# succinctlabs/sp1

Hardware: NVIDIA H100
Metric: riscv_cycles_proven_per_second_core (higher is better)
Workload: dtype u32 KoalaBear (Montgomery) / ext4

## Files before the change

sp1_b200/csrc/hostcheck.cu:

```cuda
#include "poseidon2.cuh"
#include "hostfield.hpp"
#include "zc_lower.hpp"
#include <cstring>
#include <type_traits>

extern "C" {
void sp1b200_hostcheck_permute(uint32_t* states, uint64_t n) {
    for (uint64_t i = 0; i < n; i++) {
        uint32_t s[16];
        for (int k = 0; k < 16; k++) s[k] = states[i * 16 + k];
        p2::permute(s);
        for (int k = 0; k < 16; k++) states[i * 16 + k] = s[k];
    }
}
int sp1b200_hostcheck_permute_mode(uint32_t* states, uint64_t n, int mode) {
    for (uint64_t i = 0; i < n; i++) {
        uint32_t s[16];
        for (int k = 0; k < 16; k++) s[k] = states[i * 16 + k];
        switch (mode) {
#define P2_CASE(M) case M: p2::permute_m<M>(s); break;
            P2_CASE(0) P2_CASE(1) P2_CASE(2) P2_CASE(3) P2_CASE(4) P2_CASE(5) P2_CASE(6) P2_CASE(7)
            P2_CASE(8) P2_CASE(9) P2_CASE(10) P2_CASE(11) P2_CASE(12) P2_CASE(13) P2_CASE(14) P2_CASE(15)
            P2_CASE(19) P2_CASE(21) P2_CASE(23)
#undef P2_CASE
            case -1: p2::permute_r1(s); break;
            default: return 0;
        }
        for (int k = 0; k < 16; k++) states[i * 16 + k] = s[k];
    }
    return 1;
}
void sp1b200_hostcheck_ext_mul(const uint32_t* a, const uint32_t* b, uint32_t* out, uint64_t n) {
    for (uint64_t i = 0; i < n; i++) {
        kb::Ext x{{a[4 * i], a[4 * i + 1], a[4 * i + 2], a[4 * i + 3]}}, y{{b[4 * i], b[4 * i + 1], b[4 * i + 2], b[4 * i + 3]}};
        kb::Ext r = kb::ext_mul(x, y);
        for (int k = 0; k < 4; k++) out[4 * i + k] = r.c[k];
    }
}
void sp1b200_hostcheck_ext_inv(const uint32_t* a, uint32_t* out, uint64_t n) {
    for (uint64_t i = 0; i < n; i++) {
        kb::Ext x{{a[4 * i], a[4 * i + 1], a[4 * i + 2], a[4 * i + 3]}};
        kb::Ext r = kb::ext_inv(x);
        for (int k = 0; k < 4; k++) out[4 * i + k] = r.c[k];
    }
}
void sp1b200_hostcheck_field(const uint32_t* a, const uint32_t* b, uint32_t* add, uint32_t* sub, uint32_t* mul, uint64_t n) {
    for (uint64_t i = 0; i < n; i++) { add[i] = kb::add(a[i], b[i]); sub[i] = kb::sub(a[i], b[i]); mul[i] = kb::mul(a[i], b[i]); }
}

int sp1b200_hostcheck_zc_lower(const uint32_t* chip, const uint32_t* main_row, const uint32_t* prep_row, const uint32_t* pv,
                               const uint32_t* alpha_pows, uint32_t window, uint32_t* out, uint32_t* n_lowered) {
    using hf::E4;
    const uint32_t* b = chip;
    HostProg hp;
    b += 3;
    const uint32_t n_regs = *b++;
    const uint32_t ni = *b++, nl = *b++, nc = *b++, np = *b++, na = *b++;
    hp.instrs.resize(ni); memcpy(hp.instrs.data(), b, ni * 8); b += 2 * ni;
    hp.leaves.resize(nl); memcpy(hp.leaves.data(), b, nl * 8); b += 2 * nl;
    hp.consts.assign(b, b + nc); b += nc;
    hp.publics.assign(b, b + np); b += np;
    hp.assert_regs.assign(b, b + na); b += na;
    hp.assert_alphas.assign(b, b + na); b += na;
    auto leaf = [&](const LeafRef& l) { return l.source == LEAF_MAIN ? main_row[l.col] : prep_row[l.col]; };
    {
        std::vector<uint32_t> regs(n_regs ? n_regs : 1, 0);
        for (const DagInstr& in : hp.instrs) {
            switch (in.opcode) {
                case BC_LOAD_LEAF: regs[in.out] = leaf(hp.leaves[in.a]); break;
                case BC_LOAD_CONST: regs[in.out] = hp.consts[in.a]; break;
                case BC_LOAD_PUBLIC: regs[in.out] = pv[hp.publics[in.a]]; break;
                case BC_ADD_F: regs[in.out] = hf::add(regs[in.a], regs[in.b]); break;
                case BC_SUB_F: regs[in.out] = hf::sub(regs[in.a], regs[in.b]); break;
                case BC_MUL_F: regs[in.out] = hf::mul(regs[in.a], regs[in.b]); break;
                case BC_NEG_F: regs[in.out] = hf::neg(regs[in.a]); break;
            }
        }
        E4 acc;
        for (size_t k = 0; k < hp.assert_regs.size(); k++) acc = acc + E4::load(alpha_pows + 4 * hp.assert_alphas[k]) * regs[hp.assert_regs[k]];
        acc.store(out);
    }
    auto run = [&](const ZcLowered& Lw) {
        std::vector<uint32_t> rf(Lw.n_regs, 0);
        E4 a;
        for (const ZcInstr& in : Lw.instrs) {
            switch (in.op) {
                case ZC_LOAD_MAIN: rf[in.out] = main_row[(uint32_t)in.a | ((uint32_t)in.b << 16)]; break;
                case ZC_LOAD_PREP: rf[in.out] = prep_row[(uint32_t)in.a | ((uint32_t)in.b << 16)]; break;
                case ZC_CONST: rf[in.out] = hp.consts[in.a]; break;
                case ZC_PUBLIC: rf[in.out] = pv[hp.publics[in.a]]; break;
                case ZC_ADD: { uint32_t x = rf[in.a], y = rf[in.b]; rf[in.out] = hf::add(x, y); break; }
                case ZC_SUB: { uint32_t x = rf[in.a], y = rf[in.b]; rf[in.out] = hf::sub(x, y); break; }
                case ZC_MUL: { uint32_t x = rf[in.a], y = rf[in.b]; rf[in.out] = hf::mul(x, y); break; }
                case ZC_NEG: rf[in.out] = hf::neg(rf[in.a]); break;
                case ZC_ASSERT: a = a + E4::load(alpha_pows + 4 * in.b) * rf[in.a]; break;
            }
        }
        return a;
    };
    ZcLowered L = zc_lower(hp, window);
    if (!L.error.empty()) return -1;
    if (n_lowered) *n_lowered = (uint32_t)L.instrs.size();
    E4 acc = run(L);
    {
        const size_t na = hp.assert_regs.size();
        const size_t np_ = std::max<size_t>(1, std::min<size_t>(16, na / 4));
        E4 sum;
        for (size_t q = 0; q < np_; q++) {
            ZcLowered P = zc_lower(hp, window, na * q / np_, na * (q + 1) / np_);
            if (!P.error.empty() || P.n_regs > L.n_regs + 8) return -1;
            sum = sum + run(P);
        }
        sum.store(out + 8);
    }
    acc.store(out + 4);
    return (int)L.n_regs;
}

void sp1b200_hostcheck_e4(const uint32_t* a, const uint32_t* b, uint32_t* mul_out, uint32_t* inv_out, uint64_t n) {
    using hf::E4;
    for (uint64_t i = 0; i < n; i++) {
        (E4::load(a + 4 * i) * E4::load(b + 4 * i)).store(mul_out + 4 * i);
        hf::inv(E4::load(a + 4 * i)).store(inv_out + 4 * i);
    }
}
int sp1b200_hostcheck_interpolate(const uint32_t* xs, const uint32_t* ys, uint32_t n, uint32_t* coeffs_out) {
    using hf::E4;
    auto go = [&](auto tag) {
        constexpr int N = decltype(tag)::value;
        E4 x[N], L[N][N], c[N];
        for (int i = 0; i < N; i++) x[i] = E4::load(xs + 4 * i);
        hf::lagrange_basis<N>(x, L);
        for (int k = 0; k < N; k++) for (int i = 0; i < N; i++) c[k] = c[k] + L[i][k] * E4::load(ys + 4 * i);
        for (int k = 0; k < N; k++) c[k].store(coeffs_out + 4 * k);
    };
    if (n == 3) go(std::integral_constant<int, 3>{});
    else if (n == 4) go(std::integral_constant<int, 4>{});
    else if (n == 5) go(std::integral_constant<int, 5>{});
    else return -1;
    return 0;
}
}
```

sp1_b200/csrc/zc_lower.hpp:

```cpp
#pragma once
#include "machine.cuh"
#include <cstdint>
#include <functional>
#include <queue>
#include <string>
#include <vector>

enum : uint8_t { ZC_LOAD_MAIN = 0, ZC_LOAD_PREP = 1, ZC_CONST = 2, ZC_PUBLIC = 3, ZC_ADD = 4, ZC_SUB = 5, ZC_MUL = 6, ZC_NEG = 7, ZC_ASSERT = 8 };
struct ZcInstr { uint8_t op, pad; uint16_t out, a, b; };
static_assert(sizeof(ZcInstr) == 8, "ZcInstr is one 8-byte word");

struct ZcLowered { std::vector<ZcInstr> instrs; uint32_t n_regs = 0; std::string error; };

inline ZcLowered zc_lower(const HostProg& p, uint32_t window = 24, size_t assert_begin = 0, size_t assert_end = (size_t)-1) {
    ZcLowered L;
    const size_t n = p.instrs.size();
    const int32_t NONE = -1;
    std::vector<int32_t> cur(65536, NONE);
    std::vector<int32_t> va(n, NONE), vb(n, NONE);
    std::vector<uint8_t> is_op(n, 0), needed(n, 0);
    for (size_t i = 0; i < n; i++) {
        const DagInstr& in = p.instrs[i];
        switch (in.opcode) {
            case BC_LOAD_LEAF: case BC_LOAD_CONST: case BC_LOAD_PUBLIC: break;
            case BC_ADD_F: case BC_SUB_F: case BC_MUL_F:
                va[i] = cur[in.a]; vb[i] = cur[in.b]; is_op[i] = 1;
                if (va[i] == NONE || vb[i] == NONE) { L.error = "instruction reads an undefined register"; return L; }
                break;
            case BC_NEG_F:
                va[i] = cur[in.a]; is_op[i] = 1;
                if (va[i] == NONE) { L.error = "instruction reads an undefined register"; return L; }
                break;
            default: L.error = "unknown opcode"; return L;
        }
        cur[in.out] = (int32_t)i;
    }
    std::vector<std::vector<uint32_t>> asserts_of(n);
    if (assert_end > p.assert_regs.size()) assert_end = p.assert_regs.size();
    for (size_t k = assert_begin; k < assert_end; k++) {
        const int32_t v = cur[p.assert_regs[k] & 0xffff];
        if (v == NONE) { L.error = "assert on an undefined register"; return L; }
        if (p.assert_alphas[k] > 0xffff) { L.error = "more than 65536 constraints in one chip"; return L; }
        asserts_of[v].push_back(p.assert_alphas[k]);
        needed[v] = 1;
    }
    for (size_t i = n; i-- > 0;) {
        if (!needed[i]) continue;
        if (va[i] != NONE) needed[va[i]] = 1;
        if (vb[i] != NONE) needed[vb[i]] = 1;
    }
    std::vector<uint32_t> seq;
    for (size_t i = 0; i < n; i++) if (needed[i] && is_op[i]) seq.push_back((uint32_t)i);
    std::vector<std::vector<uint32_t>> uses(n);
    for (uint32_t pos = 0; pos < seq.size(); pos++) {
        const uint32_t i = seq[pos];
        if (va[i] != NONE) uses[va[i]].push_back(pos);
        if (vb[i] != NONE && vb[i] != va[i]) uses[vb[i]].push_back(pos);
    }
    std::vector<uint32_t> use_ptr(n, 0);
    std::vector<int32_t> reg_of(n, NONE);
    std::priority_queue<uint32_t, std::vector<uint32_t>, std::greater<uint32_t>> free_regs;
    uint32_t next_reg = 0;
    auto alloc = [&]() -> uint32_t {
        if (!free_regs.empty()) { uint32_t r = free_regs.top(); free_regs.pop(); return r; }
        return next_reg++;
    };
    auto emit_load = [&](uint32_t v, uint32_t r) {
        const DagInstr& in = p.instrs[v];
        ZcInstr z{};
        z.out = (uint16_t)r;
        if (in.opcode == BC_LOAD_LEAF) {
            const LeafRef& l = p.leaves[in.a];
            z.op = l.source == LEAF_MAIN ? ZC_LOAD_MAIN : ZC_LOAD_PREP;
            z.a = (uint16_t)(l.col & 0xffff); z.b = (uint16_t)(l.col >> 16);
        } else {
            z.op = in.opcode == BC_LOAD_CONST ? ZC_CONST : ZC_PUBLIC;
            z.a = in.a;
        }
        L.instrs.push_back(z);
    };
    auto operand = [&](int32_t v) -> uint32_t {
        if (reg_of[v] == NONE) {
            reg_of[v] = (int32_t)alloc();
            emit_load((uint32_t)v, (uint32_t)reg_of[v]);
        }
        return (uint32_t)reg_of[v];
    };
    auto release_after_use = [&](int32_t v, uint32_t pos) {
        std::vector<uint32_t>& u = uses[v];
        uint32_t& q = use_ptr[v];
        while (q < u.size() && u[q] <= pos) q++;
        const bool more = q < u.size();
        const bool keep = more && (is_op[v] || u[q] - pos <= window);
        if (!keep && reg_of[v] != NONE) { free_regs.push((uint32_t)reg_of[v]); reg_of[v] = NONE; }
    };
    for (uint32_t pos = 0; pos < seq.size(); pos++) {
        const uint32_t i = seq[pos];
        const DagInstr& in = p.instrs[i];
        const uint32_t ra = operand(va[i]);
        const uint32_t rb = vb[i] != NONE ? operand(vb[i]) : 0;
        release_after_use(va[i], pos);
        if (vb[i] != NONE && vb[i] != va[i]) release_after_use(vb[i], pos);
        const uint32_t ro = alloc();
        reg_of[i] = (int32_t)ro;
        ZcInstr z{};
        z.op = in.opcode == BC_ADD_F ? ZC_ADD : in.opcode == BC_SUB_F ? ZC_SUB : in.opcode == BC_MUL_F ? ZC_MUL : ZC_NEG;
        z.out = (uint16_t)ro; z.a = (uint16_t)ra; z.b = (uint16_t)rb;
        L.instrs.push_back(z);
        for (uint32_t alpha : asserts_of[i]) L.instrs.push_back(ZcInstr{ZC_ASSERT, 0, 0, (uint16_t)ro, (uint16_t)alpha});
        if (uses[i].empty()) { free_regs.push(ro); reg_of[i] = NONE; }
    }
    for (size_t v = 0; v < n; v++) {
        if (is_op[v] || asserts_of[v].empty()) continue;
        const uint32_t r = operand((int32_t)v);
        for (uint32_t alpha : asserts_of[v]) L.instrs.push_back(ZcInstr{ZC_ASSERT, 0, 0, (uint16_t)r, (uint16_t)alpha});
        free_regs.push(r); reg_of[v] = NONE;
    }
    if (next_reg > 0xffff) { L.error = "register pressure exceeds 65535"; return L; }
    L.n_regs = next_reg ? next_reg : 1;
    return L;
}
```

sp1_b200/csrc/zerocheck.cu:

```cuda
#include "ctx.cuh"
#include "challenger.cuh"
#include "hostfield.hpp"
#include "kb31.cuh"
#include <algorithm>
#include <memory>
#include <vector>

#include "machine.cuh"
#include "zc_lower.hpp"
#include "sumcheck.cuh"

namespace {

using kb::Ext;
using hf::E4;

constexpr int ZC_BLOCK = 128;
constexpr int ZC_LOCAL_REGS = 128;
constexpr int ZC_GLOBAL_REGS = 1024;
constexpr unsigned ZC_GLOBAL_MAXB = 132 * 2;
constexpr size_t ZC_MAX_PIECES = 16;

template <class K> struct Ops;
template <> struct Ops<uint32_t> {
    static __device__ __forceinline__ uint32_t zero() { return 0; }
    static __device__ __forceinline__ uint32_t from_base(uint32_t x) { return x; }
    static __device__ __forceinline__ uint32_t add(uint32_t a, uint32_t b) { return kb::add(a, b); }
    static __device__ __forceinline__ uint32_t sub(uint32_t a, uint32_t b) { return kb::sub(a, b); }
    static __device__ __forceinline__ uint32_t mul(uint32_t a, uint32_t b) { return kb::mul(a, b); }
    static __device__ __forceinline__ uint32_t load(const uint32_t* p, uint64_t i) { return __ldg(p + i); }
    static __device__ __forceinline__ Ext scale(const Ext& e, uint32_t k) { return kb::ext_mul_base(e, k); }
};
template <> struct Ops<Ext> {
    static __device__ __forceinline__ Ext zero() { return kb::ext_zero(); }
    static __device__ __forceinline__ Ext from_base(uint32_t x) { return kb::ext_from_base(x); }
    static __device__ __forceinline__ Ext add(const Ext& a, const Ext& b) { return kb::ext_add(a, b); }
    static __device__ __forceinline__ Ext sub(const Ext& a, const Ext& b) { return kb::ext_sub(a, b); }
    static __device__ __forceinline__ Ext mul(const Ext& a, const Ext& b) { return kb::ext_mul(a, b); }
    static __device__ __forceinline__ Ext load(const Ext* p, uint64_t i) { return kb::ext_load(reinterpret_cast<const uint32_t*>(p + i)); }
    static __device__ __forceinline__ Ext scale(const Ext& e, const Ext& k) { return kb::ext_mul(e, k); }
};

struct ZcJob {
    const void* main; const void* prep; const uint32_t* alpha_pows; uint64_t h;
    uint32_t blk_start, nblk, chip, columns;
    uint32_t zc_begin, zc_end;
    const void* batch;
};
static_assert(sizeof(ZcJob) == 64, "ZcJob layout");
struct ZcFixJob {
    const void* main; const void* prep; uint32_t* out; uint64_t h;
    uint32_t main_w, prep_w, blk_start, pad;
};

template <class J>
__device__ __forceinline__ int find_job(const J* __restrict__ jobs, int n, uint32_t blk) {
    int lo = 0, hi = n - 1;
    while (lo < hi) {
        int mid = (lo + hi + 1) >> 1;
        if (jobs[mid].blk_start <= blk) lo = mid; else hi = mid - 1;
    }
    return lo;
}

enum { RF_SMEM = 0, RF_LOCAL = 1, RF_GLOBAL = 2 };
template <class K, int RF> struct RegFile;
template <class K> struct RegFile<K, RF_SMEM> {
    K* base;
    __device__ __forceinline__ RegFile(unsigned char* smem, void*, uint32_t) : base(reinterpret_cast<K*>(smem) + threadIdx.x) {}
    __device__ __forceinline__ K get(uint32_t r, int n) const { return base[(r * 3 + n) * ZC_BLOCK]; }
    __device__ __forceinline__ void set(uint32_t r, int n, const K& v) { base[(r * 3 + n) * ZC_BLOCK] = v; }
};
template <class K> struct RegFile<K, RF_LOCAL> {
    K regs[ZC_LOCAL_REGS * 3];
    __device__ __forceinline__ RegFile(unsigned char*, void*, uint32_t) {}
    __device__ __forceinline__ K get(uint32_t r, int n) const { return regs[r * 3 + n]; }
    __device__ __forceinline__ void set(uint32_t r, int n, const K& v) { regs[r * 3 + n] = v; }
};
template <class K> struct RegFile<K, RF_GLOBAL> {
    K* base;
    __device__ __forceinline__ RegFile(unsigned char*, void* ws, uint32_t ws_regs)
        : base(static_cast<K*>(ws) + (size_t)blockIdx.x * ws_regs * 3 * ZC_BLOCK + threadIdx.x) {}
    __device__ __forceinline__ K get(uint32_t r, int n) const { return base[(size_t)(r * 3 + n) * ZC_BLOCK]; }
    __device__ __forceinline__ void set(uint32_t r, int n, const K& v) { base[(size_t)(r * 3 + n) * ZC_BLOCK] = v; }
};

template <class K, int N0>
__device__ __forceinline__ void load_nodes(const K* __restrict__ base, uint32_t col, uint64_t h, uint64_t i, K (&v)[3]) {
    using O = Ops<K>;
    const K* c = base + (uint64_t)col * h;
    const K z = O::load(c, 2 * i);
    const K o = (2 * i + 1 < h) ? O::load(c, 2 * i + 1) : O::zero();
    const K d = O::sub(o, z);
    const K d2 = O::add(d, d);
    if (N0 == 0) v[0] = z;
    v[1] = O::add(z, d2);
    v[2] = O::add(v[1], d2);
}

template <class K, int RF, bool FIRST>
__global__ void __launch_bounds__(ZC_BLOCK) zc_sum_kernel(const ZcJob* __restrict__ jobs, int n_jobs, const ChipProg* __restrict__ chips,
                                                          const uint32_t* __restrict__ pv, const uint32_t* __restrict__ gkr_pows,
                                                          const uint32_t* __restrict__ E, uint32_t* __restrict__ partial,
                                                          void* __restrict__ ws, uint32_t ws_regs) {
    using O = Ops<K>;
    constexpr int N0 = FIRST ? 1 : 0;
    extern __shared__ __align__(16) unsigned char zc_smem[];
    __shared__ uint32_t red[5][4][ZC_BLOCK / 32];
    const ZcJob job = jobs[find_job(jobs, n_jobs, blockIdx.x)];
    const ChipProg& prog = chips[job.chip];
    const K* main = static_cast<const K*>(job.main);
    const K* prep = static_cast<const K*>(job.prep);
    const uint64_t h = job.h;
    const uint64_t terms = (h + 1) / 2;
    RegFile<K, RF> rf(zc_smem, ws, ws_regs);
    Ext acc[5];
#pragma unroll
    for (int a = 0; a < 5; a++) acc[a] = kb::ext_zero();
    const ZcInstr* __restrict__ zc = prog.zc + job.zc_begin;
    const uint32_t n_zc = job.zc_end - job.zc_begin;
    for (uint64_t i = (uint64_t)(blockIdx.x - job.blk_start) * ZC_BLOCK + threadIdx.x; i < terms; i += (uint64_t)job.nblk * ZC_BLOCK) {
        const Ext e = kb::ext_load(E + 4 * i);
        Ext row[3] = {kb::ext_zero(), kb::ext_zero(), kb::ext_zero()};
        ZcInstr in = n_zc ? zc[0] : ZcInstr{};
        for (uint32_t pc = 0; pc < n_zc; pc++) {
            const ZcInstr nxt = zc[pc + 1 < n_zc ? pc + 1 : pc];
            switch (in.op) {
                case ZC_LOAD_MAIN: case ZC_LOAD_PREP: {
                    K v[3];
                    load_nodes<K, N0>(in.op == ZC_LOAD_MAIN ? main : prep, (uint32_t)in.a | ((uint32_t)in.b << 16), h, i, v);
#pragma unroll
                    for (int n = N0; n < 3; n++) rf.set(in.out, n, v[n]);
                    break;
                }
                case ZC_CONST: { const K c = O::from_base(prog.consts[in.a]);
#pragma unroll
                    for (int n = N0; n < 3; n++) rf.set(in.out, n, c);
                    break; }
                case ZC_PUBLIC: { const K c = O::from_base(pv[prog.publics[in.a]]);
#pragma unroll
                    for (int n = N0; n < 3; n++) rf.set(in.out, n, c);
                    break; }
                case ZC_ADD: {
                    K r[3];
#pragma unroll
                    for (int n = N0; n < 3; n++) r[n] = O::add(rf.get(in.a, n), rf.get(in.b, n));
#pragma unroll
                    for (int n = N0; n < 3; n++) rf.set(in.out, n, r[n]);
                    break; }
                case ZC_SUB: {
                    K r[3];
#pragma unroll
                    for (int n = N0; n < 3; n++) r[n] = O::sub(rf.get(in.a, n), rf.get(in.b, n));
#pragma unroll
                    for (int n = N0; n < 3; n++) rf.set(in.out, n, r[n]);
                    break; }
                case ZC_MUL: {
                    K r[3];
#pragma unroll
                    for (int n = N0; n < 3; n++) r[n] = O::mul(rf.get(in.a, n), rf.get(in.b, n));
#pragma unroll
                    for (int n = N0; n < 3; n++) rf.set(in.out, n, r[n]);
                    break; }
                case ZC_NEG: {
                    K r[3];
#pragma unroll
                    for (int n = N0; n < 3; n++) r[n] = O::sub(O::zero(), rf.get(in.a, n));
#pragma unroll
                    for (int n = N0; n < 3; n++) rf.set(in.out, n, r[n]);
                    break; }
                case ZC_ASSERT: {
                    const Ext al = kb::ext_load(job.alpha_pows + 4 * in.b);
#pragma unroll
                    for (int n = N0; n < 3; n++) row[n] = kb::ext_add(row[n], O::scale(al, rf.get(in.a, n)));
                    break; }
                default: __trap();
            }
            in = nxt;
        }
#pragma unroll
        for (int n = N0; n < 3; n++) acc[n] = kb::ext_add(acc[n], kb::ext_mul(row[n], e));
        if (!job.columns) continue;
        Ext s0 = kb::ext_zero(), s1 = kb::ext_zero();
        const bool has_o = 2 * i + 1 < h;
        if (job.batch) {
            const uint32_t* B = static_cast<const uint32_t*>(job.batch);
            acc[3] = kb::ext_add(acc[3], kb::ext_mul(kb::ext_load(B + 8 * i), e));
            if (has_o) acc[4] = kb::ext_add(acc[4], kb::ext_mul(kb::ext_load(B + 8 * i + 4), e));
            continue;
        }
        for (uint32_t j = 0; j < prog.main_w; j++) {
            const Ext g = kb::ext_load(gkr_pows + 4 * j);
            const K* c = main + (uint64_t)j * h;
            s0 = kb::ext_add(s0, O::scale(g, O::load(c, 2 * i)));
            if (has_o) s1 = kb::ext_add(s1, O::scale(g, O::load(c, 2 * i + 1)));
        }
        for (uint32_t j = 0; j < prog.prep_w; j++) {
            const Ext g = kb::ext_load(gkr_pows + 4 * (prog.main_w + j));
            const K* c = prep + (uint64_t)j * h;
            s0 = kb::ext_add(s0, O::scale(g, O::load(c, 2 * i)));
            if (has_o) s1 = kb::ext_add(s1, O::scale(g, O::load(c, 2 * i + 1)));
        }
        acc[3] = kb::ext_add(acc[3], kb::ext_mul(s0, e));
        acc[4] = kb::ext_add(acc[4], kb::ext_mul(s1, e));
    }
    const int lane = threadIdx.x & 31, warp = threadIdx.x >> 5;
#pragma unroll
    for (int a = 0; a < 5; a++)
#pragma unroll
        for (int l = 0; l < 4; l++) {
            uint32_t v = acc[a].c[l];
            for (int s = 16; s > 0; s >>= 1) v = kb::add(v, __shfl_down_sync(0xffffffffu, v, s));
            if (lane == 0) red[a][l][warp] = v;
        }
    __syncthreads();
    if (threadIdx.x < 36) {
        const int node = threadIdx.x / 12, slot = (threadIdx.x >> 2) % 3, l = threadIdx.x & 3;
        const int a = slot == 0 ? node : (node == 0 ? 2 + slot : -1);
        uint32_t v = 0;
        if (a >= 0)
            for (int w = 0; w < ZC_BLOCK / 32; w++) v = kb::add(v, red[a][l][w]);
        partial[(uint64_t)blockIdx.x * 36 + threadIdx.x] = v;
    }
}

__global__ void __launch_bounds__(128) zc_reduce_kernel(const ZcJob* __restrict__ jobs, const uint32_t* __restrict__ partial, uint32_t* __restrict__ out,
                                                        Mail mail) {
    const ZcJob job = jobs[blockIdx.x];
    __shared__ uint32_t red[36][4];
    const int slot = threadIdx.x >> 2, part = threadIdx.x & 3;
    for (int w = slot; w < 36; w += 32) {
        uint32_t v = 0;
        for (uint32_t b = part; b < job.nblk; b += 4) v = kb::add(v, partial[(uint64_t)(job.blk_start + b) * 36 + w]);
        red[w][part] = v;
    }
    __syncthreads();
    if (threadIdx.x < 36) {
        const uint32_t* r = red[threadIdx.x];
        out[blockIdx.x * 36 + threadIdx.x] = kb::add(kb::add(r[0], r[1]), kb::add(r[2], r[3]));
    }
    sp1_mail_done(mail);
}

template <class K>
__global__ void __launch_bounds__(256) zc_fix_kernel(const ZcFixJob* __restrict__ jobs, int n_jobs, Ext alpha) {
    using O = Ops<K>;
    const ZcFixJob job = jobs[find_job(jobs, n_jobs, blockIdx.x)];
    const uint64_t h = job.h, nh = (h + 1) / 2;
    const uint32_t bpc = (uint32_t)((nh + 255) / 256);
    const uint32_t lb = blockIdx.x - job.blk_start;
    const uint64_t j = lb / bpc;
    const uint64_t i = (uint64_t)(lb - (uint32_t)j * bpc) * 256 + threadIdx.x;
    if (i >= nh) return;
    const uint64_t t = j * nh + i;
    const K* in = j < job.main_w ? static_cast<const K*>(job.main) + j * h : static_cast<const K*>(job.prep) + (j - job.main_w) * h;
    K a = O::load(in, 2 * i);
    K b = (2 * i + 1 < h) ? O::load(in, 2 * i + 1) : O::zero();
    Ext r;
    if constexpr (sizeof(K) == 4) r = kb::ext_add(kb::ext_from_base(a), kb::ext_mul_base(alpha, kb::sub(b, a)));
    else r = kb::ext_add(a, kb::ext_mul(alpha, kb::ext_sub(b, a)));
    kb::ext_store(job.out + 4 * t, r);
}

__global__ void __launch_bounds__(256) zc_batch0_kernel(const ZcFixJob* __restrict__ jobs, int n_jobs, const uint32_t* __restrict__ gkr_pows, Ext alpha) {
    const ZcFixJob job = jobs[find_job(jobs, n_jobs, blockIdx.x)];
    const uint64_t h = job.h, nh = (h + 1) / 2;
    const uint64_t i = (uint64_t)(blockIdx.x - job.blk_start) * 256 + threadIdx.x;
    if (i >= nh) return;
    const bool has_o = 2 * i + 1 < h;
    Ext sa = kb::ext_zero(), sd = kb::ext_zero();
    const uint32_t* main = static_cast<const uint32_t*>(job.main);
    const uint32_t* prep = static_cast<const uint32_t*>(job.prep);
    for (uint32_t j = 0; j < job.main_w + job.prep_w; j++) {
        const uint32_t* c = j < job.main_w ? main + (uint64_t)j * h : prep + (uint64_t)(j - job.main_w) * h;
        const uint32_t a = __ldg(c + 2 * i), b = has_o ? __ldg(c + 2 * i + 1) : 0u;
        const Ext g = kb::ext_load(gkr_pows + 4 * j);
        sa = kb::ext_add(sa, kb::ext_mul_base(g, a));
        sd = kb::ext_add(sd, kb::ext_mul_base(g, kb::sub(b, a)));
    }
    kb::ext_store(job.out + 4 * i, kb::ext_add(sa, kb::ext_mul(alpha, sd)));
}

E4 host_eval_zero_row(const HostProg& p, const uint32_t* pv, const std::vector<E4>& powers, uint32_t n_regs) {
    std::vector<uint32_t> regs(n_regs ? n_regs : 1, 0);
    for (const DagInstr& in : p.instrs) {
        switch (in.opcode) {
            case BC_LOAD_LEAF: regs[in.out] = 0; break;
            case BC_LOAD_CONST: regs[in.out] = p.consts[in.a]; break;
            case BC_LOAD_PUBLIC: regs[in.out] = pv[p.publics[in.a]]; break;
            case BC_ADD_F: regs[in.out] = hf::add(regs[in.a], regs[in.b]); break;
            case BC_SUB_F: regs[in.out] = hf::sub(regs[in.a], regs[in.b]); break;
            case BC_MUL_F: regs[in.out] = hf::mul(regs[in.a], regs[in.b]); break;
            case BC_NEG_F: regs[in.out] = hf::neg(regs[in.a]); break;
        }
// ... 11 lines not shown
        return r;
    }
    E4 at(uint64_t idx) const { return idx < threshold ? E4() : (idx == threshold ? eq_c + geq_c : geq_c); }
};

}

sp1b200_machine::~sp1b200_machine() {
    if (interactions) sp1b200_free_interactions(interactions);
    cudaFree(d_arena);
    cudaFree(d_zc_arena);
    cudaFree(d_chips);
}

extern "C" {

sp1b200_err sp1b200_machine_create(sp1b200_ctx* ctx, const uint32_t* h_blob, uint64_t n_words, sp1b200_machine** out) { SP1_DEVICE_GUARD(ctx);
    auto m = std::make_unique<sp1b200_machine>();
    SP1_CUDA(cudaMalloc((void**)&m->d_arena, n_words * 4 + 16));
    SP1_CUDA(cudaMemcpyAsync(m->d_arena, h_blob, n_words * 4, cudaMemcpyHostToDevice, ctx->stream));
    const uint32_t* b = h_blob;
    const uint32_t* end = h_blob + n_words;
    auto dev = [&](const uint32_t* hp) { return m->d_arena + (hp - h_blob); };
    if (n_words < 1 || !h_blob) return sp1b200_set_error("machine_create: empty blob");
    uint32_t n = *b++;
    for (uint32_t c = 0; c < n; c++) {
        if ((uint64_t)(end - b) < 9) return sp1b200_set_error("machine_create: truncated blob (header of chip %u)", c);
        ChipProg p{}; HostProg hp;
        p.main_w = *b++; p.prep_w = *b++; p.n_constraints = *b++; p.n_regs = *b++;
        const uint64_t ni = *b++, nl = *b++, nc = *b++, np = *b++, na = *b++;
        if (2 * ni + 2 * nl + nc + np + 2 * na > (uint64_t)(end - b)) return sp1b200_set_error("machine_create: truncated blob (chip %u)", c);
        if (p.n_regs > 65536) return sp1b200_set_error("machine_create: chip %u declares %u registers (16-bit register indices)", c, p.n_regs);
        p.n_instrs = (uint32_t)ni; p.n_asserts = (uint32_t)na;
        p.instrs = reinterpret_cast<const DagInstr*>(dev(b)); hp.instrs.resize(ni); memcpy(hp.instrs.data(), b, ni * 8); b += 2 * ni;
        p.leaves = reinterpret_cast<const LeafRef*>(dev(b)); hp.leaves.resize(nl); memcpy(hp.leaves.data(), b, nl * 8); b += 2 * nl;
        p.consts = dev(b); hp.consts.assign(b, b + nc); b += nc;
        p.publics = dev(b); hp.publics.assign(b, b + np); b += np;
        p.assert_regs = dev(b); hp.assert_regs.assign(b, b + na); b += na;
        p.assert_alphas = dev(b); hp.assert_alphas.assign(b, b + na); b += na;
        for (const LeafRef& l : hp.leaves) {
            if (l.source != LEAF_MAIN && l.source != LEAF_PREP) return sp1b200_set_error("machine_create: chip %u: leaf source %u (expected 2 = preprocessed or 4 = main)", c, l.source);
            if (l.col >= (l.source == LEAF_MAIN ? p.main_w : p.prep_w)) return sp1b200_set_error("machine_create: chip %u: leaf column %u outside the %s width", c, l.col, l.source == LEAF_MAIN ? "main" : "preprocessed");
        }
        for (size_t k = 0; k < hp.instrs.size(); k++) {
            const DagInstr& in = hp.instrs[k];
            if (in.out >= p.n_regs) return sp1b200_set_error("machine_create: chip %u instr %zu: output register %u >= n_regs %u", c, k, in.out, p.n_regs);
            bool ok = true;
            switch (in.opcode) {
                case BC_LOAD_LEAF: ok = in.a < nl; break;
                case BC_LOAD_CONST: ok = in.a < nc; break;
                case BC_LOAD_PUBLIC: ok = in.a < np; break;
                case BC_ADD_F: case BC_SUB_F: case BC_MUL_F: ok = in.a < p.n_regs && in.b < p.n_regs; break;
                case BC_NEG_F: ok = in.a < p.n_regs; break;
                default: return sp1b200_set_error("machine_create: chip %u instr %zu: unknown opcode %u", c, k, in.opcode);
            }
            if (!ok) return sp1b200_set_error("machine_create: chip %u instr %zu: operand out of range (opcode %u, a %u, b %u)", c, k, in.opcode, in.a, in.b);
        }
        for (size_t k = 0; k < hp.assert_regs.size(); k++) {
            if (hp.assert_regs[k] >= p.n_regs) return sp1b200_set_error("machine_create: chip %u assert %zu: register %u >= n_regs %u", c, k, hp.assert_regs[k], p.n_regs);
            if (hp.assert_alphas[k] >= p.n_constraints) return sp1b200_set_error("machine_create: chip %u assert %zu: alpha index %u >= n_constraints %u", c, k, hp.assert_alphas[k], p.n_constraints);
        }
        m->chips.push_back(p); m->host.push_back(std::move(hp));
    }
    {
        std::vector<uint32_t> widths;
        for (auto& c : m->chips) { widths.push_back(c.main_w); widths.push_back(c.prep_w); }
        widths.push_back(0);
        m->interactions = sp1b200_parse_interactions(b, end, n, widths.data());
        if (!m->interactions) return sp1b200_last_error();
    }
    std::vector<ZcInstr> all;
    std::vector<size_t> zc_off(n);
    for (uint32_t c = 0; c < n; c++) {
        ZcLowered L = zc_lower(m->host[c]);
        if (!L.error.empty()) return sp1b200_set_error("machine_create: chip %u: %s", c, L.error.c_str());
        zc_off[c] = all.size();
        m->chips[c].n_zc = (uint32_t)L.instrs.size();
        m->chips[c].zc_regs = L.n_regs;
        all.insert(all.end(), L.instrs.begin(), L.instrs.end());
        const size_t na = m->host[c].assert_regs.size();
        const size_t np_ = std::min<size_t>(ZC_MAX_PIECES, na / 4);
        if (np_ >= 2 && L.instrs.size() >= 128) {
            for (size_t q = 0; q < np_; q++) {
                ZcLowered P = zc_lower(m->host[c], 24, na * q / np_, na * (q + 1) / np_);
                if (!P.error.empty()) return sp1b200_set_error("machine_create: chip %u: %s", c, P.error.c_str());
                m->host[c].zc_pieces.emplace_back((uint32_t)(all.size() - zc_off[c]), (uint32_t)P.instrs.size());
                m->chips[c].zc_regs = std::max(m->chips[c].zc_regs, P.n_regs);
                all.insert(all.end(), P.instrs.begin(), P.instrs.end());
            }
        }
    }
    SP1_CUDA(cudaMalloc(&m->d_zc_arena, all.size() * sizeof(ZcInstr) + 16));
    if (!all.empty()) SP1_CUDA(cudaMemcpyAsync(m->d_zc_arena, all.data(), all.size() * sizeof(ZcInstr), cudaMemcpyHostToDevice, ctx->stream));
    for (uint32_t c = 0; c < n; c++) m->chips[c].zc = static_cast<const ZcInstr*>(m->d_zc_arena) + zc_off[c];
    SP1_CUDA(cudaMalloc((void**)&m->d_chips, (n ? n : 1) * sizeof(ChipProg)));
    if (n) SP1_CUDA(cudaMemcpyAsync(m->d_chips, m->chips.data(), n * sizeof(ChipProg), cudaMemcpyHostToDevice, ctx->stream));
    SP1_CUDA(cudaStreamSynchronize(ctx->stream));
    *out = m.release();
    return nullptr;
}
void sp1b200_machine_free(sp1b200_ctx*, sp1b200_machine* m) { delete m; }
uint32_t sp1b200_machine_chip_regs(const sp1b200_machine* m, uint32_t chip) { return chip < m->chips.size() ? m->chips[chip].zc_regs : 0; }
uint32_t sp1b200_machine_num_chips(const sp1b200_machine* m) { return (uint32_t)m->chips.size(); }

sp1b200_err sp1b200_zerocheck(sp1b200_ctx* ctx, const sp1b200_machine* m, const uint64_t* h_heights, const uint32_t* const* d_main,
                              const uint32_t* const* d_prep, const uint32_t* h_pv, uint32_t n_pv, const uint32_t* h_gkr_point,
                              const uint32_t* h_alpha, const uint32_t* h_gamma, const uint32_t* h_claims, uint32_t* h_chal, uint32_t* h_out,
                              uint64_t cap, uint64_t* h_words) { SP1_DEVICE_GUARD(ctx);
    const uint32_t mlr = ctx->params.max_log_row_count;
    const size_t nchips = m->chips.size();
    for (size_t k = 0; k < nchips; k++)
        for (uint32_t pi : m->host[k].publics)
            if (pi >= n_pv) return sp1b200_set_error("zerocheck: chip %zu reads public value %u but only %u were passed", k, pi, n_pv);
    cudaStream_t st = ctx->stream;
    DevFree mem(ctx);
    HostChallenger ch;
    SP1_TRY(ch.init(ctx, h_chal));
    PhaseTimer t_all(ctx, "zerocheck.total");
    HostAccum acc_wait(ctx, "zerocheck.host_wait"), acc_math(ctx, "zerocheck.host_math"), acc_setup(ctx, "zerocheck.host_setup");
    auto t_setup = std::make_unique<HostSpan>(acc_setup);
    const E4 alpha = E4::load(h_alpha), gamma = E4::load(h_gamma);

    struct St {
        uint64_t h;
        std::vector<E4> zeta; E4 eq_adj = E4::one(), pra; VGeq vg;
    };
    std::vector<St> S(nchips);
    size_t maxc = 0, maxw = 0, total_w = 0, total_c = 0;
    for (auto& c : m->chips) {
        maxc = std::max<size_t>(maxc, c.n_constraints); maxw = std::max<size_t>(maxw, c.main_w + c.prep_w);
        total_w += c.main_w + c.prep_w; total_c += c.n_constraints ? c.n_constraints : 1;
    }
    std::vector<E4> pw(maxc ? maxc : 1); pw[0] = E4::one();
    for (size_t i = 1; i < pw.size(); i++) pw[i] = pw[i - 1] * alpha;
    std::vector<E4> gw(maxw ? maxw : 1); gw[0] = gamma;
    for (size_t i = 1; i < gw.size(); i++) gw[i] = gw[i - 1] * gamma;
    uint32_t *d_pv, *d_gw, *d_ap;
    SP1_TRY(mem.alloc((void**)&d_pv, (n_pv ? n_pv : 1) * 4));
    if (n_pv) SP1_CUDA(cudaMemcpyAsync(d_pv, h_pv, n_pv * 4, cudaMemcpyHostToDevice, st));
    SP1_TRY(mem.alloc((void**)&d_gw, gw.size() * 16));
    SP1_CUDA(cudaMemcpyAsync(d_gw, gw.data(), gw.size() * 16, cudaMemcpyHostToDevice, st));
    std::vector<E4> gp(mlr);
    for (uint32_t i = 0; i < mlr; i++) gp[i] = E4::load(h_gkr_point + 4 * i);
    std::vector<E4> all_ap; all_ap.reserve(total_c);
    std::vector<size_t> ap_off(nchips), woff(nchips);
    std::vector<uint64_t> boff0(nchips), boff1(nchips);
    uint64_t b0 = 0, b1 = 0; size_t wsum = 0;
    for (size_t k = 0; k < nchips; k++) {
        const ChipProg& p = m->chips[k];
        St& s = S[k];
        s.h = h_heights[k];
        if (s.h > ((uint64_t)1 << mlr)) return sp1b200_set_error("zerocheck: chip %zu height exceeds 2^%u", k, mlr);
        if (p.zc_regs > ZC_GLOBAL_REGS) return sp1b200_set_error("zerocheck: chip %zu needs %u live registers (> %d)", k, p.zc_regs, ZC_GLOBAL_REGS);
        s.zeta = gp;
        std::vector<E4> rev(pw.begin(), pw.begin() + p.n_constraints);
        std::reverse(rev.begin(), rev.end());
        ap_off[k] = all_ap.size();
        all_ap.insert(all_ap.end(), rev.begin(), rev.end());
        if (rev.empty()) all_ap.push_back(E4());
        s.pra = host_eval_zero_row(m->host[k], h_pv, rev, p.n_regs);
        s.vg.threshold = (uint32_t)s.h; s.vg.geq_c = E4::one();
        const uint64_t nh = (s.h + 1) / 2;
        const size_t w = p.main_w + p.prep_w;
        boff0[k] = b0; b0 += (uint64_t)(w + 1) * nh * 4;
        boff1[k] = b1; b1 += (uint64_t)(w + 1) * ((nh + 1) / 2) * 4;
        woff[k] = wsum; wsum += w;
    }
// ... 250 lines not shown
```

Baseline: 63.61 million.

## Fold loads and asserts into zerocheck bytecode operands with forwarding

Redesigns the zerocheck bytecode. Operands now name their source directly (register, forwarded previous result, main/prep column, constant, public), so separate load instructions disappear. Results used only by the next instruction are forwarded instead of written to the register file, and assert accumulation is folded into the producing instruction via an alpha field. The per-thread accumulators move from registers to shared memory to relieve register pressure, at the cost of wider 16-byte instructions, more operand-kind branching per instruction, and repeated column loads where the old lowering kept values in a reuse window.

```diff
diff --git a/sp1_b200/csrc/hostcheck.cu b/sp1_b200/csrc/hostcheck.cu
--- a/sp1_b200/csrc/hostcheck.cu
+++ b/sp1_b200/csrc/hostcheck.cu
@@ -48,12 +48,10 @@
     for (uint64_t i = 0; i < n; i++) { add[i] = kb::add(a[i], b[i]); sub[i] = kb::sub(a[i], b[i]); mul[i] = kb::mul(a[i], b[i]); }
 }
 
-int sp1b200_hostcheck_zc_lower(const uint32_t* chip, const uint32_t* main_row, const uint32_t* prep_row, const uint32_t* pv,
-                               const uint32_t* alpha_pows, uint32_t window, uint32_t* out, uint32_t* n_lowered) {
-    using hf::E4;
-    const uint32_t* b = chip;
-    HostProg hp;
-    b += 3;
+}
+
+static uint32_t parse_chip(const uint32_t* chip, HostProg& hp) {
+    const uint32_t* b = chip + 3;
     const uint32_t n_regs = *b++;
     const uint32_t ni = *b++, nl = *b++, nc = *b++, np = *b++, na = *b++;
     hp.instrs.resize(ni); memcpy(hp.instrs.data(), b, ni * 8); b += 2 * ni;
@@ -61,7 +59,28 @@
     hp.consts.assign(b, b + nc); b += nc;
     hp.publics.assign(b, b + np); b += np;
     hp.assert_regs.assign(b, b + na); b += na;
-    hp.assert_alphas.assign(b, b + na); b += na;
+    hp.assert_alphas.assign(b, b + na);
+    return n_regs;
+}
+
+extern "C" {
+int sp1b200_hostcheck_zc_stream(const uint32_t* chip, uint64_t assert_begin, uint64_t assert_end, uint32_t* instrs_out, uint64_t cap,
+                                uint64_t* n_instrs) {
+    HostProg hp;
+    parse_chip(chip, hp);
+    ZcLowered L = zc_lower(hp, assert_begin, assert_end);
+    if (!L.error.empty()) return -1;
+    if (n_instrs) *n_instrs = L.instrs.size();
+    if (instrs_out) memcpy(instrs_out, L.instrs.data(), std::min<uint64_t>(cap, L.instrs.size()) * sizeof(ZcInstr));
+    return (int)L.n_regs;
+}
+
+int sp1b200_hostcheck_zc_lower(const uint32_t* chip, const uint32_t* main_row, const uint32_t* prep_row, const uint32_t* pv,
+                               const uint32_t* alpha_pows, uint32_t window, uint32_t* out, uint32_t* n_lowered) {
+    using hf::E4;
+    (void)window;
+    HostProg hp;
+    const uint32_t n_regs = parse_chip(chip, hp);
     auto leaf = [&](const LeafRef& l) { return l.source == LEAF_MAIN ? main_row[l.col] : prep_row[l.col]; };
     {
         std::vector<uint32_t> regs(n_regs ? n_regs : 1, 0);
@@ -80,25 +99,43 @@
         for (size_t k = 0; k < hp.assert_regs.size(); k++) acc = acc + E4::load(alpha_pows + 4 * hp.assert_alphas[k]) * regs[hp.assert_regs[k]];
         acc.store(out);
     }
+    bool bad = false;
     auto run = [&](const ZcLowered& Lw) {
         std::vector<uint32_t> rf(Lw.n_regs, 0);
+        uint32_t fwd = 0;
+        bool have_fwd = false;
         E4 a;
+        auto operand = [&](uint32_t kind, uint32_t idx) -> uint32_t {
+            switch (kind) {
+                case ZC_OPD_REG: if (idx < rf.size()) return rf[idx]; break;
+                case ZC_OPD_FWD: if (have_fwd) return fwd; break;
+                case ZC_OPD_MAIN: return main_row[idx];
+                case ZC_OPD_PREP: return prep_row[idx];
+                case ZC_OPD_CONST: if (idx < hp.consts.size()) return hp.consts[idx]; break;
+                case ZC_OPD_PUBLIC: if (idx < hp.publics.size()) return pv[hp.publics[idx]]; break;
+            }
+            bad = true;
+            return 0;
+        };
         for (const ZcInstr& in : Lw.instrs) {
+            const uint32_t x = operand(zc_kind_a(in), in.a);
+            const uint32_t y = in.op <= ZC_MUL ? operand(zc_kind_b(in), in.b) : 0;
+            uint32_t r = 0;
             switch (in.op) {
-                case ZC_LOAD_MAIN: rf[in.out] = main_row[(uint32_t)in.a | ((uint32_t)in.b << 16)]; break;
-                case ZC_LOAD_PREP: rf[in.out] = prep_row[(uint32_t)in.a | ((uint32_t)in.b << 16)]; break;
-                case ZC_CONST: rf[in.out] = hp.consts[in.a]; break;
-                case ZC_PUBLIC: rf[in.out] = pv[hp.publics[in.a]]; break;
-                case ZC_ADD: { uint32_t x = rf[in.a], y = rf[in.b]; rf[in.out] = hf::add(x, y); break; }
-                case ZC_SUB: { uint32_t x = rf[in.a], y = rf[in.b]; rf[in.out] = hf::sub(x, y); break; }
-                case ZC_MUL: { uint32_t x = rf[in.a], y = rf[in.b]; rf[in.out] = hf::mul(x, y); break; }
-                case ZC_NEG: rf[in.out] = hf::neg(rf[in.a]); break;
-                case ZC_ASSERT: a = a + E4::load(alpha_pows + 4 * in.b) * rf[in.a]; break;
+                case ZC_ADD: r = hf::add(x, y); break;
+                case ZC_SUB: r = hf::sub(x, y); break;
+                case ZC_MUL: r = hf::mul(x, y); break;
+                case ZC_NEG: r = hf::neg(x); break;
+                case ZC_MOV: r = x; break;
+                default: bad = true;
             }
+            if (zc_res(in) == ZC_RES_FILE) { if (in.out < rf.size()) rf[in.out] = r; else bad = true; }
+            if (in.alpha) a = a + E4::load(alpha_pows + 4 * (in.alpha - 1)) * r;
+            fwd = r; have_fwd = true;
         }
         return a;
     };
-    ZcLowered L = zc_lower(hp, window);
+    ZcLowered L = zc_lower(hp);
     if (!L.error.empty()) return -1;
     if (n_lowered) *n_lowered = (uint32_t)L.instrs.size();
     E4 acc = run(L);
@@ -107,14 +144,14 @@
         const size_t np_ = std::max<size_t>(1, std::min<size_t>(16, na / 4));
         E4 sum;
         for (size_t q = 0; q < np_; q++) {
-            ZcLowered P = zc_lower(hp, window, na * q / np_, na * (q + 1) / np_);
+            ZcLowered P = zc_lower(hp, na * q / np_, na * (q + 1) / np_);
             if (!P.error.empty() || P.n_regs > L.n_regs + 8) return -1;
             sum = sum + run(P);
         }
         sum.store(out + 8);
     }
     acc.store(out + 4);
-    return (int)L.n_regs;
+    return bad ? -1 : (int)L.n_regs;
 }
 
 void sp1b200_hostcheck_e4(const uint32_t* a, const uint32_t* b, uint32_t* mul_out, uint32_t* inv_out, uint64_t n) {
diff --git a/sp1_b200/csrc/zc_lower.hpp b/sp1_b200/csrc/zc_lower.hpp
--- a/sp1_b200/csrc/zc_lower.hpp
+++ b/sp1_b200/csrc/zc_lower.hpp
@@ -6,13 +6,23 @@
 #include <string>
 #include <vector>
 
-enum : uint8_t { ZC_LOAD_MAIN = 0, ZC_LOAD_PREP = 1, ZC_CONST = 2, ZC_PUBLIC = 3, ZC_ADD = 4, ZC_SUB = 5, ZC_MUL = 6, ZC_NEG = 7, ZC_ASSERT = 8 };
-struct ZcInstr { uint8_t op, pad; uint16_t out, a, b; };
-static_assert(sizeof(ZcInstr) == 8, "ZcInstr is one 8-byte word");
+enum : uint8_t { ZC_ADD = 0, ZC_SUB = 1, ZC_MUL = 2, ZC_NEG = 3, ZC_MOV = 4 };
+enum : uint8_t { ZC_OPD_REG = 0, ZC_OPD_FWD = 1, ZC_OPD_MAIN = 2, ZC_OPD_PREP = 3, ZC_OPD_CONST = 4, ZC_OPD_PUBLIC = 5 };
+enum : uint8_t { ZC_RES_FILE = 0, ZC_RES_FWD = 1, ZC_RES_NONE = 2 };
+struct alignas(16) ZcInstr {
+    uint8_t op, kinds;
+    uint16_t out;
+    uint32_t a, b;
+    uint32_t alpha;
+};
+static_assert(sizeof(ZcInstr) == 16, "ZcInstr is one 16-byte word");
+inline uint32_t zc_kind_a(const ZcInstr& z) { return z.kinds & 7; }
+inline uint32_t zc_kind_b(const ZcInstr& z) { return (z.kinds >> 3) & 7; }
+inline uint32_t zc_res(const ZcInstr& z) { return z.kinds >> 6; }
 
 struct ZcLowered { std::vector<ZcInstr> instrs; uint32_t n_regs = 0; std::string error; };
 
-inline ZcLowered zc_lower(const HostProg& p, uint32_t window = 24, size_t assert_begin = 0, size_t assert_end = (size_t)-1) {
+inline ZcLowered zc_lower(const HostProg& p, size_t assert_begin = 0, size_t assert_end = (size_t)-1) {
     ZcLowered L;
     const size_t n = p.instrs.size();
     const int32_t NONE = -1;
@@ -40,7 +50,7 @@
     for (size_t k = assert_begin; k < assert_end; k++) {
         const int32_t v = cur[p.assert_regs[k] & 0xffff];
         if (v == NONE) { L.error = "assert on an undefined register"; return L; }
-        if (p.assert_alphas[k] > 0xffff) { L.error = "more than 65536 constraints in one chip"; return L; }
+        if (p.assert_alphas[k] >= 0xffffffffu) { L.error = "alpha index out of range"; return L; }
         asserts_of[v].push_back(p.assert_alphas[k]);
         needed[v] = 1;
     }
@@ -57,7 +67,6 @@
         if (va[i] != NONE) uses[va[i]].push_back(pos);
         if (vb[i] != NONE && vb[i] != va[i]) uses[vb[i]].push_back(pos);
     }
-    std::vector<uint32_t> use_ptr(n, 0);
     std::vector<int32_t> reg_of(n, NONE);
     std::priority_queue<uint32_t, std::vector<uint32_t>, std::greater<uint32_t>> free_regs;
     uint32_t next_reg = 0;
@@ -65,56 +74,56 @@
         if (!free_regs.empty()) { uint32_t r = free_regs.top(); free_regs.pop(); return r; }
         return next_reg++;
     };
-    auto emit_load = [&](uint32_t v, uint32_t r) {
+    int32_t fwd = NONE;
+    auto operand = [&](int32_t v, uint32_t& idx) -> uint8_t {
+        idx = 0;
+        if (v == fwd) return ZC_OPD_FWD;
+        if (is_op[v]) { idx = (uint32_t)reg_of[v]; return ZC_OPD_REG; }
         const DagInstr& in = p.instrs[v];
-        ZcInstr z{};
-        z.out = (uint16_t)r;
         if (in.opcode == BC_LOAD_LEAF) {
             const LeafRef& l = p.leaves[in.a];
-            z.op = l.source == LEAF_MAIN ? ZC_LOAD_MAIN : ZC_LOAD_PREP;
-            z.a = (uint16_t)(l.col & 0xffff); z.b = (uint16_t)(l.col >> 16);
-        } else {
-            z.op = in.opcode == BC_LOAD_CONST ? ZC_CONST : ZC_PUBLIC;
-            z.a = in.a;
+            idx = l.col;
+            return l.source == LEAF_MAIN ? ZC_OPD_MAIN : ZC_OPD_PREP;
         }
-        L.instrs.push_back(z);
-    };
-    auto operand = [&](int32_t v) -> uint32_t {
-        if (reg_of[v] == NONE) {
-            reg_of[v] = (int32_t)alloc();
-            emit_load((uint32_t)v, (uint32_t)reg_of[v]);
-        }
-        return (uint32_t)reg_of[v];
+        idx = in.a;
+        return in.opcode == BC_LOAD_CONST ? ZC_OPD_CONST : ZC_OPD_PUBLIC;
     };
     auto release_after_use = [&](int32_t v, uint32_t pos) {
-        std::vector<uint32_t>& u = uses[v];
-        uint32_t& q = use_ptr[v];
-        while (q < u.size() && u[q] <= pos) q++;
-        const bool more = q < u.size();
-        const bool keep = more && (is_op[v] || u[q] - pos <= window);
-        if (!keep && reg_of[v] != NONE) { free_regs.push((uint32_t)reg_of[v]); reg_of[v] = NONE; }
+        if (is_op[v] && reg_of[v] != NONE && uses[v].back() == pos) { free_regs.push((uint32_t)reg_of[v]); reg_of[v] = NONE; }
+    };
+    auto more_asserts = [&](int32_t v) {
+        for (size_t k = 1; k < asserts_of[v].size(); k++)
+            L.instrs.push_back(ZcInstr{ZC_MOV, (uint8_t)(ZC_OPD_FWD | ZC_RES_NONE << 6), 0, 0, 0, asserts_of[v][k] + 1});
     };
     for (uint32_t pos = 0; pos < seq.size(); pos++) {
         const uint32_t i = seq[pos];
         const DagInstr& in = p.instrs[i];
-        const uint32_t ra = operand(va[i]);
-        const uint32_t rb = vb[i] != NONE ? operand(vb[i]) : 0;
+        ZcInstr z{};
+        z.op = in.opcode == BC_ADD_F ? ZC_ADD : in.opcode == BC_SUB_F ? ZC_SUB : in.opcode == BC_MUL_F ? ZC_MUL : ZC_NEG;
+        const uint8_t ka = operand(va[i], z.a);
+        const uint8_t kb = vb[i] != NONE ? operand(vb[i], z.b) : 0;
         release_after_use(va[i], pos);
         if (vb[i] != NONE && vb[i] != va[i]) release_after_use(vb[i], pos);
-        const uint32_t ro = alloc();
-        reg_of[i] = (int32_t)ro;
-        ZcInstr z{};
-        z.op = in.opcode == BC_ADD_F ? ZC_ADD : in.opcode == BC_SUB_F ? ZC_SUB : in.opcode == BC_MUL_F ? ZC_MUL : ZC_NEG;
-        z.out = (uint16_t)ro; z.a = (uint16_t)ra; z.b = (uint16_t)rb;
+        const std::vector<uint32_t>& u = uses[i];
+        uint8_t res = ZC_RES_FILE;
+        if (u.empty()) res = ZC_RES_NONE;
+        else if (u.size() == 1 && u[0] == pos + 1) res = ZC_RES_FWD;
+        else { reg_of[i] = (int32_t)alloc(); z.out = (uint16_t)reg_of[i]; }
+        z.kinds = (uint8_t)(ka | kb << 3 | res << 6);
+        z.alpha = asserts_of[i].empty() ? 0 : asserts_of[i][0] + 1;
         L.instrs.push_back(z);
-        for (uint32_t alpha : asserts_of[i]) L.instrs.push_back(ZcInstr{ZC_ASSERT, 0, 0, (uint16_t)ro, (uint16_t)alpha});
-        if (uses[i].empty()) { free_regs.push(ro); reg_of[i] = NONE; }
+        fwd = (int32_t)i;
+        more_asserts((int32_t)i);
     }
     for (size_t v = 0; v < n; v++) {
         if (is_op[v] || asserts_of[v].empty()) continue;
-        const uint32_t r = operand((int32_t)v);
-        for (uint32_t alpha : asserts_of[v]) L.instrs.push_back(ZcInstr{ZC_ASSERT, 0, 0, (uint16_t)r, (uint16_t)alpha});
-        free_regs.push(r); reg_of[v] = NONE;
+        ZcInstr z{};
+        z.op = ZC_MOV;
+        z.kinds = (uint8_t)(operand((int32_t)v, z.a) | ZC_RES_NONE << 6);
+        z.alpha = asserts_of[v][0] + 1;
+        L.instrs.push_back(z);
+        fwd = (int32_t)v;
+        more_asserts((int32_t)v);
     }
     if (next_reg > 0xffff) { L.error = "register pressure exceeds 65535"; return L; }
     L.n_regs = next_reg ? next_reg : 1;
diff --git a/sp1_b200/csrc/zerocheck.cu b/sp1_b200/csrc/zerocheck.cu
--- a/sp1_b200/csrc/zerocheck.cu
+++ b/sp1_b200/csrc/zerocheck.cu
@@ -98,6 +98,31 @@
     v[2] = O::add(v[1], d2);
 }
 
+template <class K, int N0, class RFile>
+__device__ __forceinline__ void zc_operand(uint32_t kind, uint32_t idx, const RFile& rf, const K (&fwd)[3], const K* __restrict__ main,
+                                           const K* __restrict__ prep, const ChipProg& prog, const uint32_t* __restrict__ pv, uint64_t h,
+                                           uint64_t i, K (&v)[3]) {
+    using O = Ops<K>;
+    switch (kind) {
+        case ZC_OPD_REG:
+#pragma unroll
+            for (int n = N0; n < 3; n++) v[n] = rf.get(idx, n);
+            break;
+        case ZC_OPD_FWD:
+#pragma unroll
+            for (int n = N0; n < 3; n++) v[n] = fwd[n];
+            break;
+        case ZC_OPD_MAIN: load_nodes<K, N0>(main, idx, h, i, v); break;
+        case ZC_OPD_PREP: load_nodes<K, N0>(prep, idx, h, i, v); break;
+        default: {
+            const K c = O::from_base(kind == ZC_OPD_CONST ? prog.consts[idx] : pv[prog.publics[idx]]);
+#pragma unroll
+            for (int n = N0; n < 3; n++) v[n] = c;
+            break;
+        }
+    }
+}
+
 template <class K, int RF, bool FIRST>
 __global__ void __launch_bounds__(ZC_BLOCK) zc_sum_kernel(const ZcJob* __restrict__ jobs, int n_jobs, const ChipProg* __restrict__ chips,
                                                           const uint32_t* __restrict__ pv, const uint32_t* __restrict__ gkr_pows,
@@ -114,79 +139,71 @@
     const uint64_t h = job.h;
     const uint64_t terms = (h + 1) / 2;
     RegFile<K, RF> rf(zc_smem, ws, ws_regs);
-    Ext acc[5];
-#pragma unroll
-    for (int a = 0; a < 5; a++) acc[a] = kb::ext_zero();
+    __shared__ uint32_t acc_s[5][4][ZC_BLOCK];
+    auto acc_add = [&](int a, const Ext& v) {
+#pragma unroll
+        for (int l = 0; l < 4; l++) acc_s[a][l][threadIdx.x] = kb::add(acc_s[a][l][threadIdx.x], v.c[l]);
+    };
+#pragma unroll
+    for (int a = 0; a < 5; a++)
+#pragma unroll
+        for (int l = 0; l < 4; l++) acc_s[a][l][threadIdx.x] = 0;
     const ZcInstr* __restrict__ zc = prog.zc + job.zc_begin;
     const uint32_t n_zc = job.zc_end - job.zc_begin;
     for (uint64_t i = (uint64_t)(blockIdx.x - job.blk_start) * ZC_BLOCK + threadIdx.x; i < terms; i += (uint64_t)job.nblk * ZC_BLOCK) {
-        const Ext e = kb::ext_load(E + 4 * i);
         Ext row[3] = {kb::ext_zero(), kb::ext_zero(), kb::ext_zero()};
+        K fwd[3] = {O::zero(), O::zero(), O::zero()};
         ZcInstr in = n_zc ? zc[0] : ZcInstr{};
         for (uint32_t pc = 0; pc < n_zc; pc++) {
             const ZcInstr nxt = zc[pc + 1 < n_zc ? pc + 1 : pc];
+            K x[3], y[3], r[3];
+            zc_operand<K, N0>(in.kinds & 7, in.a, rf, fwd, main, prep, prog, pv, h, i, x);
+            if (in.op <= ZC_MUL) zc_operand<K, N0>((in.kinds >> 3) & 7, in.b, rf, fwd, main, prep, prog, pv, h, i, y);
             switch (in.op) {
-                case ZC_LOAD_MAIN: case ZC_LOAD_PREP: {
-                    K v[3];
-                    load_nodes<K, N0>(in.op == ZC_LOAD_MAIN ? main : prep, (uint32_t)in.a | ((uint32_t)in.b << 16), h, i, v);
-#pragma unroll
-                    for (int n = N0; n < 3; n++) rf.set(in.out, n, v[n]);
+                case ZC_ADD:
+#pragma unroll
+                    for (int n = N0; n < 3; n++) r[n] = O::add(x[n], y[n]);
                     break;
-                }
-                case ZC_CONST: { const K c = O::from_base(prog.consts[in.a]);
-#pragma unroll
-                    for (int n = N0; n < 3; n++) rf.set(in.out, n, c);
-                    break; }
-                case ZC_PUBLIC: { const K c = O::from_base(pv[prog.publics[in.a]]);
-#pragma unroll
-                    for (int n = N0; n < 3; n++) rf.set(in.out, n, c);
-                    break; }
-                case ZC_ADD: {
-                    K r[3];
-#pragma unroll
-                    for (int n = N0; n < 3; n++) r[n] = O::add(rf.get(in.a, n), rf.get(in.b, n));
-#pragma unroll
-                    for (int n = N0; n < 3; n++) rf.set(in.out, n, r[n]);
-                    break; }
-                case ZC_SUB: {
-                    K r[3];
-#pragma unroll
-                    for (int n = N0; n < 3; n++) r[n] = O::sub(rf.get(in.a, n), rf.get(in.b, n));
-#pragma unroll
-                    for (int n = N0; n < 3; n++) rf.set(in.out, n, r[n]);
-                    break; }
-                case ZC_MUL: {
-                    K r[3];
-#pragma unroll
-                    for (int n = N0; n < 3; n++) r[n] = O::mul(rf.get(in.a, n), rf.get(in.b, n));
-#pragma unroll
-                    for (int n = N0; n < 3; n++) rf.set(in.out, n, r[n]);
-                    break; }
-                case ZC_NEG: {
-                    K r[3];
-#pragma unroll
-                    for (int n = N0; n < 3; n++) r[n] = O::sub(O::zero(), rf.get(in.a, n));
-#pragma unroll
-                    for (int n = N0; n < 3; n++) rf.set(in.out, n, r[n]);
-                    break; }
-                case ZC_ASSERT: {
-                    const Ext al = kb::ext_load(job.alpha_pows + 4 * in.b);
-#pragma unroll
-                    for (int n = N0; n < 3; n++) row[n] = kb::ext_add(row[n], O::scale(al, rf.get(in.a, n)));
-                    break; }
+                case ZC_SUB:
+#pragma unroll
+                    for (int n = N0; n < 3; n++) r[n] = O::sub(x[n], y[n]);
+                    break;
+                case ZC_MUL:
+#pragma unroll
+                    for (int n = N0; n < 3; n++) r[n] = O::mul(x[n], y[n]);
+                    break;
+                case ZC_NEG:
+#pragma unroll
+                    for (int n = N0; n < 3; n++) r[n] = O::sub(O::zero(), x[n]);
+                    break;
+                case ZC_MOV:
+#pragma unroll
+                    for (int n = N0; n < 3; n++) r[n] = x[n];
+                    break;
                 default: __trap();
             }
+            if ((in.kinds >> 6) == ZC_RES_FILE)
+#pragma unroll
+                for (int n = N0; n < 3; n++) rf.set(in.out, n, r[n]);
+            if (in.alpha) {
+                const Ext al = kb::ext_load(job.alpha_pows + 4 * (in.alpha - 1));
+#pragma unroll
+                for (int n = N0; n < 3; n++) row[n] = kb::ext_add(row[n], O::scale(al, r[n]));
+            }
+#pragma unroll
+            for (int n = N0; n < 3; n++) fwd[n] = r[n];
             in = nxt;
         }
-#pragma unroll
-        for (int n = N0; n < 3; n++) acc[n] = kb::ext_add(acc[n], kb::ext_mul(row[n], e));
+        const Ext e = kb::ext_load(E + 4 * i);
+#pragma unroll
+        for (int n = N0; n < 3; n++) acc_add(n, kb::ext_mul(row[n], e));
         if (!job.columns) continue;
         Ext s0 = kb::ext_zero(), s1 = kb::ext_zero();
         const bool has_o = 2 * i + 1 < h;
         if (job.batch) {
             const uint32_t* B = static_cast<const uint32_t*>(job.batch);
-            acc[3] = kb::ext_add(acc[3], kb::ext_mul(kb::ext_load(B + 8 * i), e));
-            if (has_o) acc[4] = kb::ext_add(acc[4], kb::ext_mul(kb::ext_load(B + 8 * i + 4), e));
+            acc_add(3, kb::ext_mul(kb::ext_load(B + 8 * i), e));
+            if (has_o) acc_add(4, kb::ext_mul(kb::ext_load(B + 8 * i + 4), e));
             continue;
         }
         for (uint32_t j = 0; j < prog.main_w; j++) {
@@ -201,15 +218,15 @@
             s0 = kb::ext_add(s0, O::scale(g, O::load(c, 2 * i)));
             if (has_o) s1 = kb::ext_add(s1, O::scale(g, O::load(c, 2 * i + 1)));
         }
-        acc[3] = kb::ext_add(acc[3], kb::ext_mul(s0, e));
-        acc[4] = kb::ext_add(acc[4], kb::ext_mul(s1, e));
+        acc_add(3, kb::ext_mul(s0, e));
+        acc_add(4, kb::ext_mul(s1, e));
     }
     const int lane = threadIdx.x & 31, warp = threadIdx.x >> 5;
 #pragma unroll
     for (int a = 0; a < 5; a++)
 #pragma unroll
         for (int l = 0; l < 4; l++) {
-            uint32_t v = acc[a].c[l];
+            uint32_t v = acc_s[a][l][threadIdx.x];
             for (int s = 16; s > 0; s >>= 1) v = kb::add(v, __shfl_down_sync(0xffffffffu, v, s));
             if (lane == 0) red[a][l][warp] = v;
         }
@@ -387,7 +404,7 @@
         const size_t np_ = std::min<size_t>(ZC_MAX_PIECES, na / 4);
         if (np_ >= 2 && L.instrs.size() >= 128) {
             for (size_t q = 0; q < np_; q++) {
-                ZcLowered P = zc_lower(m->host[c], 24, na * q / np_, na * (q + 1) / np_);
+                ZcLowered P = zc_lower(m->host[c], na * q / np_, na * (q + 1) / np_);
                 if (!P.error.empty()) return sp1b200_set_error("machine_create: chip %u: %s", c, P.error.c_str());
                 m->host[c].zc_pieces.emplace_back((uint32_t)(all.size() - zc_off[c]), (uint32_t)P.instrs.size());
                 m->chips[c].zc_regs = std::max(m->chips[c].zc_regs, P.n_regs);
```

Result: faster. 64.81 million (median of 6 runs) (+1.9%).
